# XiangLi2022/CM-TTS

Measured on AMD Instinct MI355X. Metric: mel-frames/s (text->mel hot path, consistency sampling T=4), higher is better.
Workload: dtype f32

## Files before the change

cm-tts_amd/csrc/cmtts_api.hip:

```cpp
#include <hip/hip_runtime.h>
#include <limits.h>
#include <math.h>
#include <stdio.h>
#include <stdlib.h>
#include <string.h>

#include <algorithm>
#include <map>
#include <string>
#include <vector>

#include "../../include/cmtts_hip.h"
#include "internal_hooks.h"
#include "conv_args.h"
#include "kernels.h"
#include "resblock_args.h"
#include "persist_args.h"
#include "cond_gemm.h"
#include "resblock_pair.h"
#include "inproj.h"
#include "attention.h"
#include "text_state.h"

namespace {
// ... 1046 lines not shown
}

struct FrameWs {
    float *xlr, *h128, *hp, *c1, *c2, *cwt, *r, *s1, *s2, *stats, *f0;
    int64_t* pidx;
    size_t bytes;
};
FrameWs carve_frame(const cmtts_config& c, int B, int T, void* base) {
    Carver cv(base);
    FrameWs w;
    const size_t n = (size_t)B * c.hidden * T;
    w.xlr = cv.take<float>(n);
    w.h128 = cv.take<float>((size_t)B * c.cwt_hidden * T);
    w.hp = cv.take<float>((size_t)B * c.cwt_hidden * T);
    w.c1 = cv.take<float>(n);
    w.c2 = cv.take<float>(n);
    w.cwt = cv.take<float>((size_t)B * T * 16);
    w.r = cv.take<float>((size_t)B * T);
    w.s1 = cv.take<float>((size_t)B * c.cwt_hidden);
    w.s2 = cv.take<float>((size_t)B * c.cwt_hidden);
    w.stats = cv.take<float>((size_t)B * 2);
    w.f0 = cv.take<float>((size_t)B * T);
    w.pidx = cv.take<int64_t>((size_t)B * T);
    w.bytes = cv.off + 256;
    return w;
}

struct DenWs {
    float *hin, *h, *u, *zb, *skip, *emb, *e1, *e2, *dproj, *sproj, *dp, *tbuf, *xcur, *cp;
    float* pst;
    unsigned long long* halo;
    size_t bytes;
};
DenWs carve_den(const cmtts_config& c, int B, int T, void* base) {
    Carver cv(base);
    DenWs w;
    const int C = c.res_channels, NL = c.res_layers;
    const size_t n = (size_t)B * C * T;
    w.hin = cv.take<float>((size_t)B * c.n_mels * T);
    w.h = cv.take<float>(n);
    w.u = cv.take<float>(n);
    w.zb = cv.take<float>(n);
    w.skip = cv.take<float>(n);
    w.emb = cv.take<float>((size_t)B * C);
    w.e1 = cv.take<float>((size_t)B * 4 * C);
    w.e2 = cv.take<float>((size_t)B * C);
    w.dproj = cv.take<float>((size_t)B * NL * C);
    w.sproj = cv.take<float>((size_t)B * NL * C);
    w.dp = cv.take<float>((size_t)B * NL * C);
    w.tbuf = cv.take<float>((size_t)B);
    w.xcur = cv.take<float>((size_t)B * T * c.n_mels);
    w.cp = cv.take<float>((size_t)NL * n);
    w.halo = cv.take<unsigned long long>(cmtts_persist_halo_bytes(B, T) / sizeof(unsigned long long));
    w.pst = cv.take<float>(cmtts_persist_state_floats(B, T));
    w.bytes = cv.off + 256;
    return w;
}

struct EnergyHead {
    const float* xin; const float* e_target; float e_control; const float* bins; int nbins; const float* E; float* out1; int64_t* e_idx; float* e_scaled;
    bool done;
};
int g_energy_head = 1;
int g_pred_wino = 1;
int g_pred_xres = 1;
int predictor(const Predictor& P, const float* in, int ld_in, int B, int T, int ld, const int64_t* ln_lens,
              const int64_t* out_lens, float* bufA, float* bufB, float* out, int O, hipStream_t s, int mode16 = 0, bool frame_level = false,
              EnergyHead* eh = nullptr) {
    const float* cur = in;
    int ldc = ld_in;
    auto other = [&](const float* p) { return p == bufA ? bufB : bufA; };
    int pend_ln = -1;
    for (size_t li = 0; li < P.convs.size(); ++li) {
        const PackedConv& w = P.convs[li];
        int rx = -2;
        float* dst = other(cur);
        if (frame_level && !mode16 && g_pred_wino && !ln_lens && li < P.convs_q.size() && P.convs_q[li] && w.taps == 5 && w.cout == 256 &&
            (pend_ln < 0 || w.cin == 256)) {
            ConvXlArgs xa;
            memset(&xa, 0, sizeof(xa));
            xa.x = cur; xa.y = dst; xa.wf = P.convs_q[li]; xa.bias = w.bias; xa.bstride = (long)w.cout * ld;
            xa.B = B; xa.C = 256; xa.T = T; xa.ld = ld; xa.k = w.taps; xa.dil = 1; xa.slope = 1.0f; xa.relu = 1;
            if (w.cin != 256) { xa.cin = w.cin; xa.xbstride = (long)w.cin * ldc; }
            if (pend_ln >= 0) { xa.ln_g = P.ln_g[pend_ln]; xa.ln_b = P.ln_b[pend_ln]; xa.ln_eps = 1e-12f; }
            if (ldc == ld || w.cin != 256) {
                rx = cmtts_launch_conv_k5q(&xa, (void*)s);
                if (rx == -3) return fail(CMTTS_E_HIP, "conv_k5q launch failed");
                if (rx == 0) pend_ln = -2;
            }
        }
        const bool small = (long)((T + 63) / 64) * B < 192;
        if (rx != 0 && !mode16 && g_pred_xres && small && P.convs_f[li] && w.cin == 256 && w.cout == 256 && ldc == ld) {
            ConvArgs a = conv_args(w, cur, T, ldc, (long)w.cin * ldc, dst, ld, (long)w.cout * ld, T);
            a.out[0].act = ACT_RELU;
            a.xres_nt = 1;
            if (pend_ln >= 0) { a.ln_g = P.ln_g[pend_ln]; a.ln_b = P.ln_b[pend_ln]; a.ln_eps = 1e-12f; a.ln_lens = ln_lens; a.ln_skip_tiles = 1; }
            rx = cmtts_launch_conv_xres(&a, P.convs_f[li], B, (void*)s);
            if (rx == -3) return fail(CMTTS_E_HIP, "conv_xres launch failed");
            if (rx == 0) pend_ln = -2;
        }
        if (pend_ln >= 0) {
            float* nd = other(cur);
            k_layernorm_ct(cur, nd, P.ln_g[pend_ln], P.ln_b[pend_ln], 1e-12f, ln_lens, B, T, ld, s);
            cur = nd;
            dst = other(cur);
        }
        pend_ln = -1;
        if (mode16 && li < P.convs_f16[mode16 - 1].size() && P.convs_f16[mode16 - 1][li]) {
            ConvArgs a = conv_args(w, cur, T, ldc, (long)w.cin * ldc, dst, ld, (long)w.cout * ld, T);
            a.out[0].act = ACT_RELU;
            a.text_epi = 1;
            rx = cmtts_launch_conv16(&a, P.convs_f16[mode16 - 1][li], mode16, B, (void*)s);
            if (rx == -3) return fail(CMTTS_E_HIP, "text16: predictor conv launch failed");
        }
        if (rx != 0 && g_pred_xl && P.convs_f[li] && ldc == ld && (long)((T + 63) / 64) * B >= 192) {
            ConvXlArgs xa;
            memset(&xa, 0, sizeof(xa));
            xa.x = cur; xa.y = dst; xa.wf = P.convs_f[li]; xa.bias = w.bias; xa.bstride = (long)w.cout * ld;
            xa.B = B; xa.C = 256; xa.T = T; xa.ld = ld; xa.k = w.taps; xa.dil = 1; xa.slope = 1.0f; xa.relu = 1;
            if (w.cin != 256) { xa.cin = w.cin; xa.xbstride = (long)w.cin * ldc; }
            rx = cmtts_launch_conv_xl(&xa, (void*)s);
            if (rx == -3) return fail(CMTTS_E_HIP, "conv_xl launch failed");
        }
        if (rx != 0) {
            ConvArgs a = conv_args(w, cur, T, ldc, (long)w.cin * ldc, dst, ld, (long)w.cout * ld, T);
            a.out[0].act = ACT_RELU;
            CHK(launch(a, EPI_PLAIN, B, s));
        }
        cur = dst;
        ldc = ld;
        if (g_pred_head && eh && g_energy_head && O == 1 && li + 1 == P.convs.size() && w.cout == 256) {
            k_ln_linear_energy(cur, P.ln_g[li], P.ln_b[li], 1e-12f, P.lin_w, P.lin_b, out, ln_lens, out_lens, B, T, ld, eh->xin, eh->e_target, eh->e_control,
                               eh->bins, eh->nbins, eh->E, eh->out1, eh->e_idx, eh->e_scaled, s);
            eh->done = true;
            return 0;
        }
        if (g_pred_head && li + 1 == P.convs.size() && w.cout == 256 &&
            k_ln_linear(cur, P.ln_g[li], P.ln_b[li], 1e-12f, P.lin_w, P.lin_b, out, ln_lens, out_lens, B, T, ld, O, s))
            return 0;
        pend_ln = (int)li;
    }
    if (pend_ln >= 0) {
        float* nd = other(cur);
        k_layernorm_ct(cur, nd, P.ln_g[pend_ln], P.ln_b[pend_ln], 1e-12f, ln_lens, B, T, ld, s);
        cur = nd;
    }
    k_chan_linear(cur, P.lin_w, P.lin_b, out, out_lens, B, P.convs.back().cout, T, ld, O, s);
    return 0;
}

int cond_projections(cmtts_model* m, const DenWs& w, const float* cond_ct, int B, int T, hipStream_t s) {
    const cmtts_config& c = m->cfg;
    if (g_cond_gemm16 && m->precision >= 1 && m->precision <= 3 && m->cond_all_f16[m->precision - 1]) {
        CondGemmArgs g;
        g.X = cond_ct; g.Wf = nullptr; g.bias = m->cond_all.bias; g.Y = w.cp;
        g.row_split = 0;
        g.B = B; g.T = T; g.M = c.res_layers * c.res_channels; g.K = c.hidden; g.force = 1;
        const int r = cmtts_launch_cond_gemm16(&g, m->cond_all_f16[m->precision - 1], m->precision, (void*)s);
        if (r == 0) return 0;
        if (r != -2) return fail(CMTTS_E_HIP, "cond_gemm16 launch failed");
    }
    if (m->cond_all_f) {
        CondGemmArgs g;
        g.X = cond_ct; g.Wf = m->cond_all_f; g.bias = m->cond_all.bias; g.Y = w.cp;
        g.row_split = 0;
        g.B = B; g.T = T; g.M = c.res_layers * c.res_channels; g.K = c.hidden; g.force = g_cond_gemm == 2;
        const int r = g_cond_gemm ? cmtts_launch_cond_gemm(&g, (void*)s) : -2;
        if (r == 0) return 0;
        if (r != -2) return fail(CMTTS_E_HIP, "cond_gemm launch failed");
    }
    ConvArgs a = conv_args(m->cond_all, cond_ct, T, T, (long)c.hidden * T, w.cp, T, (long)c.res_layers * c.res_channels * T, T);
    return launch(a, EPI_PLAIN, B, s);
}

struct CondFactors {
    const float* p1 = nullptr;
    const float* p1t = nullptr;
    int ldp = 0, L = 0;
    const int64_t* mel2ph = nullptr;
    const int64_t* p_idx = nullptr;
    bool usable(const cmtts_model* m) const;
};
int g_cond_factored = 1;
int g_cond_inkernel = 1;
inline bool C_IS_256(const cmtts_config& c) { return c.res_channels == 256; }
bool CondFactors::usable(const cmtts_model* m) const {
    return g_cond_factored && p1 && mel2ph && p_idx && m->precision == 0 && m->cond_p2 && g_fused_resblock;
}
int cond_factored(cmtts_model* m, const DenWs& w, const CondFactors& f, int B, int T, hipStream_t s) {
    const cmtts_config& c = m->cfg;
    const int r = cmtts_launch_cond_expand(f.p1, f.ldp, f.L, m->cond_p2, c.pitch_bins, f.mel2ph, f.p_idx, w.cp, B, c.res_layers * c.res_channels, T, (void*)s);
    return r == 0 ? 0 : fail(CMTTS_E_HIP, "cond_expand launch failed");
}
int cond_phoneme_factor(cmtts_model* m, const float* out1, int B, int Lp, float* p1, hipStream_t s) {
    const cmtts_config& c = m->cfg;
    if (!m->cond_p2) return fail(CMTTS_E_UNSUPPORTED, "factored conditioner projections are not available for this model");
    CondGemmArgs g;
    memset(&g, 0, sizeof(g));
    g.X = out1; g.Wf = m->cond_all_f; g.bias = m->cond_zero_bias; g.Y = p1;
    g.B = B; g.T = Lp; g.M = c.res_layers * c.res_channels; g.K = c.hidden; g.force = 1;
    g.flat = 1;
    const long tiles = ((long)B * Lp + 63) / 64;
    const int npass = g.M / 512;
    int best = 1;
    double best_t = 1e30;
    for (int sp = 1; sp <= npass; ++sp) {
        const int ppg = (npass + sp - 1) / sp, groups = (npass + ppg - 1) / ppg;
        const long wg = tiles * groups, cap = persist_blocks();
        const double t = (double)((wg + cap - 1) / cap) * ppg;
        if (t < best_t - 1e-9) { best_t = t; best = sp; }
    }
    g.row_split = best;
    const int r = cmtts_launch_cond_gemm(&g, (void*)s);
    return r == 0 ? 0 : fail(r == -2 ? CMTTS_E_UNSUPPORTED : CMTTS_E_HIP, "cond_gemm (phoneme factor) launch failed");
}

int step_embedding(cmtts_model* m, const DenWs& w, const float* timesteps, const float* spk, int B, hipStream_t s,
                   float t_host = NAN) {
    const cmtts_config& c = m->cfg;
    const int C = c.res_channels, NL = c.res_layers;
    if (c.multi_speaker && !spk) return fail(CMTTS_E_INVALID, "speaker_emb is required for a multi-speaker model");
    const bool cacheable = g_step_cache && t_host == t_host;
    if (cacheable) {
        for (const cmtts_model::StepRow& e : m->step_rows)
            if (e.t == t_host && hipEventQuery(e.ready) == hipSuccess) {
                k_broadcast_row(e.row, w.dproj, B, NL * C, s);
                if (c.multi_speaker) {
                    k_dense_small(spk, c.hidden, 1, m->sproj_wt, nullptr, nullptr, w.sproj, B, c.hidden, NL * C, DENSE_NONE, s);
                    k_add_rows(w.dproj, w.sproj, w.dp, (long)B * NL * C, s);
                }
                return 0;
            }
    }
    k_diff_embed(timesteps, m->omega_res, w.emb, B, C, s);
    k_dense_small(w.emb, C, 1, m->mlp0_wt, nullptr, nullptr, w.e1, B, C, 4 * C, DENSE_MISH, s);
    k_dense_small(w.e1, 4 * C, 1, m->mlp2_wt, nullptr, nullptr, w.e2, B, 4 * C, C, DENSE_NONE, s);
    k_dense_small(w.e2, C, 1, m->dproj_wt, nullptr, nullptr, w.dproj, B, C, NL * C, DENSE_NONE, s);
    if (c.multi_speaker) {
        k_dense_small(spk, c.hidden, 1, m->sproj_wt, nullptr, nullptr, w.sproj, B, c.hidden, NL * C, DENSE_NONE, s);
        k_dense_small(w.e2, C, 1, m->dproj_wt, nullptr, w.sproj, w.dp, B, C, NL * C, DENSE_NONE, s);
    }
    if (cacheable && m->step_rows.size() < 16) {
        bool known = false;
        for (const cmtts_model::StepRow& e : m->step_rows) known = known || e.t == t_host;
        if (!known) {
            cmtts_model::StepRow e{t_host, nullptr, nullptr};
            void* p = nullptr;
            if (hipMalloc(&p, (size_t)NL * C * sizeof(float)) == hipSuccess && hipEventCreateWithFlags(&e.ready, hipEventDisableTiming) == hipSuccess) {
                e.row = (float*)p;
                m->al.ptrs.push_back(p);
                HIPCHK(hipMemcpyAsync(e.row, w.dproj, (size_t)NL * C * sizeof(float), hipMemcpyDeviceToDevice, s));
                HIPCHK(hipEventRecord(e.ready, s));
                m->step_rows.push_back(e);
            } else if (p) {
                (void)hipFree(p);
            }
        }
    }
    return 0;
}

struct MelPost {
    const float* xold;
    const float* noise;
    float c_out, c_skip, nstd;
    float* out;
};

int denoiser_prologue(cmtts_model* m, const DenWs& w, const float* x_src, float in_scale, const float* timesteps, const float* spk, int B,
                      int T, hipStream_t s, bool embed, float t_host, bool* halo_zeroed) {
    const cmtts_config& c = m->cfg;
    const int C = c.res_channels, NL = c.res_layers, M = c.n_mels;
    const long cs = (long)C * T;
    *halo_zeroed = false;
    int rin = -2;
    if (g_inproj_fused && m->in_proj_f) {
        InProjArgs ia;
        memset(&ia, 0, sizeof(ia));
        ia.x = x_src; ia.scale = in_scale; ia.wf = m->in_proj_f; ia.bias = m->in_proj.bias; ia.h = w.h;
        ia.B = B; ia.T = T; ia.M = M; ia.C = C;
        const bool persist_path = g_fused_resblock && g_persist && NL <= PERSIST_MAX_LAYERS;
        if (persist_path) { ia.zero = w.halo; ia.zero_f4 = (long)(cmtts_persist_halo_bytes(B, T) / 16); }
        rin = cmtts_launch_inproj(&ia, (void*)s);
        if (rin == -3) return fail(CMTTS_E_HIP, "inproj launch failed");
        *halo_zeroed = rin == 0 && persist_path && cmtts_persist_halo_bytes(B, T) % 16 == 0;
    }
    if (rin != 0) {
        k_mel_prep(x_src, nullptr, in_scale, w.hin, B, T, M, s);
        ConvArgs a = conv_args(m->in_proj, w.hin, T, T, (long)M * T, w.h, T, cs, T);
        a.out[0].act = ACT_RELU;
        CHK(launch(a, EPI_PLAIN, B, s));
    }
    if (embed) CHK(step_embedding(m, w, timesteps, spk, B, s, t_host));
    return 0;
}

int denoiser_core(cmtts_model* m, const DenWs& w, const float* x_src, float in_scale, const float* timesteps,
                  const float* cond_ct, const float* spk, int B, int T, const MelPost& post, hipStream_t s, bool embed = true,
                  SideStream* pending = nullptr, float t_host = NAN,
                  const CondFactors* cfk = nullptr, bool* cp_ready = nullptr) {
    CHK(check_device_flag(true));
    const cmtts_config& c = m->cfg;
    const int C = c.res_channels, NL = c.res_layers, M = c.n_mels;
    const long cs = (long)C * T;
    bool halo_zeroed = false;
    CHK(denoiser_prologue(m, w, x_src, in_scale, timesteps, spk, B, T, s, embed, t_host, &halo_zeroed));
    if (pending) CHK(branch_join(pending));
    const float* dp = m->cfg.multi_speaker ? w.dp : w.dproj;
    const bool unfused = !g_fused_resblock;
    float* hcur = w.h;
    float* halt = w.u;
    bool layers_done = false;
    if (!unfused && g_persist && NL <= PERSIST_MAX_LAYERS) {
        PersistArgs pa;
        memset(&pa, 0, sizeof(pa));
        pa.x0 = w.h; pa.cp = w.cp; pa.cp_bstride = (long)NL * C * T;
        pa.dp = dp; pa.d = w.dproj; pa.vec_stride = (long)NL * C;
        pa.skip = w.skip; pa.halo = w.halo; pa.tmo = g_tmo_host;
        pa.B = B; pa.T = T; pa.NL = NL;
        pa.halo_zeroed = halo_zeroed;
        const int prec = m->precision;
        if (cfk && !(cp_ready && *cp_ready)) {
            pa.fact = 1; pa.p1 = cfk->p1; pa.p2 = m->cond_p2; pa.mel2ph = (const long long*)cfk->mel2ph; pa.pidx = (const long long*)cfk->p_idx;
            pa.ldp = cfk->ldp; pa.Lph = cfk->L; pa.ld2 = c.pitch_bins;
            pa.p1t = cfk->p1t; pa.p2t = m->cond_p2t;
        }
        if (g_persist_tail && m->skip_f && m->outp_f) {
            pa.tail = 1;
            pa.Wsf = m->skip_f; pa.bs = m->skip_proj.bias; pa.Wpf = m->outp_f; pa.bp = m->out_proj.bias;
            pa.skip_div = (float)sqrt((double)NL); pa.n_mels = M;
            pa.xold = post.xold; pa.noise = post.noise; pa.c_out = post.c_out; pa.c_skip = post.c_skip; pa.nstd = post.nstd;
            pa.out = post.out;
        }
        pa.wino = g_persist_wino && m->winograd && !prec && m->res[0].w3w && w.pst;
        if (pa.wino && g_persist_wino == 3 && m->winograd == 1 && m->res[0].w3w43) pa.wino = 3;
        pa.xst = w.pst;
        for (int l = 0; l < NL; ++l) {
            pa.W3f[l] = prec ? (const float*)m->res[l].w3f16[prec - 1] : (pa.wino == 3 ? m->res[l].w3w43 : pa.wino ? m->res[l].w3w : m->res[l].w3f);
            pa.Wof[l] = prec ? (const float*)m->res[l].wof16[prec - 1] : m->res[l].wof;
            pa.b3[l] = m->res[l].b3f; pa.bo[l] = m->res[l].outp.bias;
        }
        const bool prof = g_prof.on && g_prof.used + 2 <= g_prof.ev.size();
        const int need = cmtts_persist_plan(B, T, NL, persist_blocks(), g_persist == 2);
        if (need) CHK(persist_admit(s, need, persist_blocks()));
        if (prof) (void)hipEventRecord(g_prof.ev[g_prof.used], s);
        const int rc = prec ? cmtts_launch_denoiser_persist_lp(&pa, prec, persist_blocks(), g_persist == 2, (void*)s)
                            : cmtts_launch_denoiser_persist(&pa, persist_blocks(), g_persist == 2, (void*)s);
        if (rc == -3) return fail(CMTTS_E_HIP, "persistent denoiser launch failed");
        if (rc == 0) {
            CHK(persist_launched(s, need));
            if (prof) { (void)hipEventRecord(g_prof.ev[g_prof.used + 1], s); g_prof.used += 2; }
            layers_done = true;
            if (pa.tail) return 0;
        }
    }
    if (!layers_done && cfk && !(cp_ready && *cp_ready)) {
        CHK(cond_factored(m, w, *cfk, B, T, s));
        if (cp_ready) *cp_ready = true;
    }
    for (int l = 0; l < NL && !layers_done; ++l) {
        const ResLayer& R = m->res[l];
        const bool prof = g_prof.on && g_prof.used + 2 <= g_prof.ev.size() && (g_prof.seen++ % g_prof.stride) == 0;
        if (!unfused) {
            ResArgs ra;
            memset(&ra, 0, sizeof(ra));
            ra.x_in = hcur; ra.cp = w.cp + (long)l * C * T; ra.cp_bstride = (long)NL * C * T;
// ... 237 lines not shown
            ConvArgs a = conv_args(E.ffn1, ln_ffn ? w.x : w.h, L, Lp, hs, w.f, Lp, 4 * hs, L);
            a.out[0].alpha = (float)pow((double)c.ffn_kernel, -0.5);
            a.out[0].act = ACT_GELU_ERF;
            if (ln_ffn) { a.ln_g = E.ln2_g; a.ln_b = E.ln2_b; a.ln_eps = 1e-12f; a.ln_lens = pad_lens; a.ln_skip_tiles = pad_lens != nullptr; }
            int rc = -2;
            if (xr && g_ffn_fused && ffn2_seg && E.ffn2_f && E.ffn1.cout == FFN2_SEG * 128) {
                a.w2frag = E.ffn2_f; a.part = w.part; a.part_zs0 = (long)FFN2_SEG * hs; a.part_zs1 = hs; a.part_ld = Lp; a.M2 = H;
                rc = wq ? cmtts_launch_conv_xresq(&a, wqf, B, (void*)s, g_ffn_wino == 2 ? 1 : 2) : -2;
                if (rc == -2) rc = cmtts_launch_conv_xres(&a, E.ffn1_f, B, (void*)s);
                if (rc == 0) ffn_fused = true;
                else { a.w2frag = nullptr; a.part = nullptr; }
            }
            if (xr && !ffn_fused) rc = cmtts_launch_conv_xres(&a, E.ffn1_f, B, (void*)s);
            if (rc == -3) return fail(CMTTS_E_HIP, "conv_xres launch failed");
            if (rc != 0) {
                if (ln_ffn) {
                    k_layernorm_ct(w.x, w.h, E.ln2_g, E.ln2_b, 1e-12f, pad_lens, B, L, Lp, s);
                    a.X = w.h; a.ln_g = a.ln_b = nullptr; a.ln_lens = nullptr;
                }
                CHK(launch(a, EPI_PLAIN, B, s));
            }
        }
        if (ffn_fused) {
            k_reduce_partials(w.part, FFN2_SEG, E.ffn2.bias, w.x, src_lens, w.x, B, H, L, Lp, s);
        } else if (ffn2_seg) {
            const int kseg = E.ffn2.cin / FFN2_SEG;
            ConvArgs a = conv_args(E.ffn2, w.f, L, Lp, 4 * hs, w.part, Lp, (long)FFN2_SEG * hs, L);
            a.K = kseg;
            a.zdiv = FFN2_SEG; a.a_zs0 = 0; a.a_zs1 = (long)kseg * a.a_ld; a.x_zs1 = (long)kseg * Lp;
            a.out[0].y_zs1 = hs; a.out[0].bias = nullptr;
            CHK(launch(a, EPI_PLAIN, B * FFN2_SEG, s));
            k_reduce_partials(w.part, FFN2_SEG, E.ffn2.bias, w.x, src_lens, w.x, B, H, L, Lp, s);
        } else {
            ConvArgs a = conv_args(E.ffn2, w.f, L, Lp, 4 * hs, w.x, Lp, hs, L);
            a.out[0].res = w.x; a.out[0].r_zs0 = hs; a.out[0].ldr = Lp; a.out[0].lens = src_lens;
            CHK(launch(a, EPI_PLAIN, B, s));
        }
    }
    return 0;
}

int cmtts_text_forward(cmtts_model* m, const int64_t* texts, const int64_t* src_lens, const float* spker_embeds,
                       const int64_t* speakers, int B, int L, float d_control, float* log_d, float* d_rounded, int64_t* mel_len,
                       float* e_pred, int64_t* e_idx, float* enc_out_ct, float* speaker_emb,
                       void* text_ws, size_t text_ws_bytes, void* stream) {
    return cmtts_text_forward_ragged(m, texts, src_lens, nullptr, spker_embeds, speakers, B, L, d_control, log_d, d_rounded, mel_len, e_pred,
                                     e_idx, enc_out_ct, speaker_emb, text_ws, text_ws_bytes, stream);
}

int cmtts_text_forward_ragged(cmtts_model* m, const int64_t* texts, const int64_t* src_lens, const int64_t* pad_lens, const float* spker_embeds,
                              const int64_t* speakers, int B, int L, float d_control, float* log_d, float* d_rounded, int64_t* mel_len,
                              float* e_pred, int64_t* e_idx, float* enc_out_ct, float* speaker_emb,
                              void* text_ws, size_t text_ws_bytes, void* stream) {
    if (!m || !m->finalized) return fail(CMTTS_E_INVALID, "model not finalized");
    if (!texts || !src_lens || !text_ws || B <= 0 || L <= 0) return fail(CMTTS_E_INVALID, "cmtts_text_forward: bad argument");
    const cmtts_config& c = m->cfg;
    if (c.multi_speaker && c.n_speaker > 0 && !speakers) return fail(CMTTS_E_INVALID, "speakers (ids into the speaker_emb table) are required (model/cmtts.py:78)");
    if (c.multi_speaker && c.n_speaker <= 0 && !spker_embeds) return fail(CMTTS_E_INVALID, "Speaker embedding should not be None (model/cmtts.py:80)");
    TextWs w = carve_text(c, B, L, text_ws);
    if (text_ws_bytes < w.bytes) return fail(CMTTS_E_WORKSPACE, "text workspace too small");
    hipStream_t s = (hipStream_t)stream;
    const int H = c.hidden, Lp = round_up(L, 4);
    if (!log_d) log_d = w.logd;
    if (!d_rounded) d_rounded = w.dround;
    if (!mel_len) mel_len = w.mlen;
    if (!e_pred) e_pred = w.epred;
    if (!e_idx) e_idx = w.eidx;

    k_embed_tokens(texts, src_lens, m->embed, m->omega_h, m->pe_h, PE_ROWS, w.x, B, L, Lp, H, (float)sqrt((double)H), s);
    CHK(fft_stack(m, m->enc, w, src_lens, B, L, s, pad_lens));
    k_layernorm_ct(w.x, w.x, m->encln_g, m->encln_b, 1e-5f, src_lens, B, L, Lp, s);
    if (enc_out_ct && c.multi_speaker)
        k_copy_rows(enc_out_ct, L, w.x, Lp, L, (long)B * H, s);
    if (c.multi_speaker) {
        if (c.n_speaker > 0) k_gather_rows(m->spk_table, speakers, w.spk, B, H, c.n_speaker, s);
        else k_dense_small(spker_embeds, c.external_speaker_dim, 1, m->spk_wt, m->spk_b, nullptr, w.spk, B,
                      c.external_speaker_dim, H, DENSE_NONE, s);
        k_add_rowvec(w.x, w.spk, B, H, L, Lp, s, pad_lens);
        if (speaker_emb) HIPCHK(hipMemcpyAsync(speaker_emb, w.spk, (size_t)B * H * 4, hipMemcpyDeviceToDevice, s));
    }
    SideStream* ss = side_for(s);
    hipStream_t se = ss ? ss->side : s;
    float* ec1 = ss ? w.qk : w.c1;
    float* ec2 = ss ? w.qk + (size_t)B * H * Lp : w.c2;
    if (ss) CHK(branch_fork(ss));
    const int t16mode = (m->text16 && (m->precision == 1 || m->precision == 2)) ? m->precision : 0;
    CHK(predictor(m->dur, w.x, Lp, B, L, Lp, src_lens, src_lens, w.c1, w.c2, log_d, 1, s, t16mode));
    if (m->vc.d_target) {
        HIPCHK(hipMemcpyAsync(d_rounded, m->vc.d_target, (size_t)B * L * 4, hipMemcpyDeviceToDevice, s));
        k_cumsum_durations(m->vc.d_target, w.cum, mel_len, B, L, s);
    } else {
        k_durations(log_d, d_control, d_rounded, w.cum, mel_len, B, L, s);
    }
    if (enc_out_ct && !c.multi_speaker)
        k_copy_rows(enc_out_ct, L, w.x, Lp, L, (long)B * H, s);
    k_pos_embed_add(w.x, w.h, m->energy.alpha, m->omega_h, m->pe_h, PE_ROWS, B, H, L, Lp, se);
    EnergyHead eh{w.x, m->vc.e_target, m->vc.e_control, m->energy_bins, c.energy_bins - 1, m->energy_emb, w.out1, e_idx, w.escaled, false};
    CHK(predictor(m->energy, w.h, Lp, B, L, Lp, pad_lens, pad_lens, ec1, ec2, e_pred, 1, se, t16mode, false, H == 256 ? &eh : nullptr));
    if (ss) CHK(branch_join(ss));
    if (!eh.done)
        k_energy_embed(w.x, e_pred, w.escaled, m->vc.e_target, m->vc.e_control, m->energy_bins, c.energy_bins - 1, m->energy_emb,
                       w.out1, e_idx, B, H, L, Lp, s);
    {
        ConvArgs a = conv_args(m->cwt_in, w.out1, L, Lp, (long)H * Lp, w.h128, Lp, (long)c.cwt_hidden * Lp, L);
        int rc = -2;
        if (g_ffn_xres && g_pred_xres && m->cwt_in_f) {
            a.xres_nt = 1;
            rc = cmtts_launch_conv_xres(&a, m->cwt_in_f, B, (void*)s);
            if (rc == -3) return fail(CMTTS_E_HIP, "conv_xres launch failed");
            a.xres_nt = 0;
        }
        if (rc != 0) CHK(launch(a, EPI_PLAIN, B, s));
    }
    if (!m->vc.e_target && m->vc.e_control != 1.0f)
        HIPCHK(hipMemcpyAsync(e_pred, w.escaled, (size_t)B * L * 4, hipMemcpyDeviceToDevice, s));
    HIPCHK(hipGetLastError());
    return 0;
}

int cmtts_frame_forward(cmtts_model* m, const void* text_ws, int B, int L, int T, float* cond_ct, int64_t* mel2ph,
                        float* cwt_out, float* f0_denorm, int64_t* p_idx, float* f0_stats, void* frame_ws,
                        size_t frame_ws_bytes, void* stream) {
    return cmtts_frame_forward_sub(m, text_ws, B, L, 0, B, T, cond_ct, mel2ph, cwt_out, f0_denorm, p_idx, f0_stats, nullptr, frame_ws, frame_ws_bytes, stream);
}

int cmtts_frame_forward_sub(cmtts_model* m, const void* text_ws, int B_all, int L_all, int b0, int B, int T, float* cond_ct, int64_t* mel2ph,
                            float* cwt_out, float* f0_denorm, int64_t* p_idx, float* f0_stats, float* cond_p1, void* frame_ws,
                            size_t frame_ws_bytes, void* stream) {
    return cmtts_frame_forward_sub_t(m, text_ws, B_all, L_all, b0, B, T, cond_ct, mel2ph, cwt_out, f0_denorm, p_idx, f0_stats, cond_p1, nullptr, frame_ws,
                                     frame_ws_bytes, stream);
}

int cmtts_frame_forward_sub_t(cmtts_model* m, const void* text_ws, int B_all, int L_all, int b0, int B, int T, float* cond_ct, int64_t* mel2ph,
                              float* cwt_out, float* f0_denorm, int64_t* p_idx, float* f0_stats, float* cond_p1, float* cond_p1t, void* frame_ws,
                              size_t frame_ws_bytes, void* stream) {
    if (!m || !m->finalized) return fail(CMTTS_E_INVALID, "model not finalized");
    if (!text_ws || !frame_ws || !cond_ct || !mel2ph || B <= 0 || L_all <= 0 || T <= 0 || b0 < 0 || b0 + B > B_all)
        return fail(CMTTS_E_INVALID, "cmtts_frame_forward: bad argument");
    const cmtts_config& c = m->cfg;
    const int L = L_all;
    TextWs tw = carve_text(c, B_all, L_all, const_cast<void*>(text_ws));
    tw.out1 += (size_t)b0 * c.hidden * round_up(L_all, 4);
    tw.h128 += (size_t)b0 * c.cwt_hidden * round_up(L_all, 4);
    tw.cum += (size_t)b0 * L_all;
    FrameWs w = carve_frame(c, B, T, frame_ws);
    if (frame_ws_bytes < w.bytes) return fail(CMTTS_E_WORKSPACE, "frame workspace too small");
    hipStream_t s = (hipStream_t)stream;
    const int H = c.hidden, Lp = round_up(L, 4), O = c.use_uv ? 11 : 10, CH = c.cwt_hidden;
    if (!cwt_out) cwt_out = w.cwt;
    if (!f0_denorm) f0_denorm = w.f0;
    if (!p_idx) p_idx = w.pidx;
    if (!f0_stats) f0_stats = w.stats;

    SideStream* ss = side_for(s);
    hipStream_t sst = ss ? ss->side : s;
    if (ss) CHK(branch_fork(ss));
    if (cond_p1t && !cond_p1) return fail(CMTTS_E_INVALID, "cmtts_frame_forward_sub_t: cond_p1t needs cond_p1");
    if (cond_p1 && m->cond_p2) {
        CHK(cond_phoneme_factor(m, tw.out1, B, Lp, cond_p1, sst));
        if (cond_p1t) k_transpose(cond_p1, cond_p1t, B * c.res_layers, c.res_channels, Lp, sst);
    }
    if (!(g_stats_mlp && k_stats_mlp(tw.out1, (long)H * Lp, Lp, m->st0_wt, m->st0_b, m->st2_wt, m->st2_b, m->st4_wt, m->st4_b, f0_stats, B, H, CH, CH, 2, sst))) {
        k_dense_small(tw.out1, (long)H * Lp, Lp, m->st0_wt, m->st0_b, nullptr, w.s1, B, H, CH, DENSE_RELU, sst);
        k_dense_small(w.s1, CH, 1, m->st2_wt, m->st2_b, nullptr, w.s2, B, CH, CH, DENSE_RELU, sst);
        k_dense_small(w.s2, CH, 1, m->st4_wt, m->st4_b, nullptr, f0_stats, B, CH, 2, DENSE_NONE, sst);
    }
    k_mel2ph(tw.cum, mel2ph, B, L, T, s);
    if (!g_cwt_in_phoneme) k_length_regulate(tw.out1, mel2ph, w.xlr, B, H, Lp, T, s);
    bool hp_done = false;
    if (g_cwt_in_phoneme) {
        k_pos_embed_add_lr(tw.h128, Lp, mel2ph, m->cwt_in.bias, w.hp, m->cwt.alpha, m->omega_cwt, m->pe_cwt, PE_ROWS, B, CH, T, s);
        hp_done = true;
    } else {
        ConvArgs a = conv_args(m->cwt_in, w.xlr, T, T, (long)H * T, w.h128, T, (long)CH * T, T);
        CHK(launch(a, EPI_PLAIN, B, s));
    }
    if (!hp_done) k_pos_embed_add(w.h128, w.hp, m->cwt.alpha, m->omega_cwt, m->pe_cwt, PE_ROWS, B, CH, T, T, s);
    CHK(predictor(m->cwt, w.hp, T, B, T, T, nullptr, nullptr, w.c1, w.c2, cwt_out, O, s, (m->text16 && (m->precision == 1 || m->precision == 2)) ? m->precision : 0, true));
    if (ss) CHK(branch_join(ss));
    if (m->vc.p_control != 1.0f) k_scale(cwt_out, cwt_out, (long)B * T * O, m->vc.p_control, s);
    if (m->vc.cwt_spec) {
        k_pitch_index(m->vc.cwt_spec, 10, m->vc.f0_mean, m->vc.f0_std, 1, 1.0f, nullptr, 0, c.use_uv ? m->vc.uv : nullptr,
                      c.pitch_norm_eps, w.r, p_idx, f0_denorm, B, T, s);
    } else {
        k_pitch_index(cwt_out, O, f0_stats, f0_stats + 1, 2, c.cwt_std_scale, c.use_uv ? cwt_out + (O - 1) : nullptr, O, nullptr,
                      c.pitch_norm_eps, w.r, p_idx, f0_denorm, B, T, s);
    }
    if (g_cwt_in_phoneme) k_lr_gather_add(tw.out1, mel2ph, Lp, p_idx, m->pitch_emb, cond_ct, B, H, T, s);
    else k_gather_add(w.xlr, p_idx, m->pitch_emb, cond_ct, B, H, T, s);
    HIPCHK(hipGetLastError());
    return 0;
}

namespace {
struct TextStateLayout {
    long off[TEXT_STATE_MAX_REGIONS], bytes[TEXT_STATE_MAX_REGIONS], stride[TEXT_STATE_MAX_REGIONS];
    long rec_bytes;
};
TextStateLayout text_state_layout(const cmtts_config& c, int L) {
    const int Lp = round_up(L, 4);
    TextStateLayout t;
    t.bytes[0] = (long)c.hidden * Lp * 4;
    t.bytes[1] = (long)c.cwt_hidden * Lp * 4;
    t.bytes[2] = (long)c.hidden * 4;
    t.bytes[3] = (long)L * 4;
    long off = TEXT_STATE_HEADER_BYTES;
    for (int g = 0; g < TEXT_STATE_MAX_REGIONS; ++g) {
        t.stride[g] = t.bytes[g];
        t.off[g] = off;
        off += (t.bytes[g] + 15) / 16 * 16;
    }
    t.rec_bytes = off;
    return t;
}
TextStateCopy text_state_args(const cmtts_config& c, void* ws, int B_all, int L, void* records, int n, int unpack) {
    const TextStateLayout t = text_state_layout(c, L);
    TextWs tw = carve_text(c, B_all, L, ws);
    char* base[TEXT_STATE_MAX_REGIONS] = {(char*)tw.out1, (char*)tw.h128, (char*)tw.spk, (char*)tw.cum};
    TextStateCopy a;
    memset(&a, 0, sizeof(a));
    int chunks = 0;
    for (int g = 0; g < TEXT_STATE_MAX_REGIONS; ++g) {
        TextStateRegion& R = a.reg[g];
        R.ws = base[g]; R.ws_stride = t.stride[g]; R.rec_off = t.off[g]; R.bytes = t.bytes[g];
        R.vec16 = ((uintptr_t)R.ws % 16 == 0 && R.ws_stride % 16 == 0 && R.bytes % 16 == 0 && (uintptr_t)records % 16 == 0) ? 1 : 0;
        R.chunk0 = chunks;
        chunks += (int)((R.bytes + TEXT_STATE_CHUNK - 1) / TEXT_STATE_CHUNK);
    }
    a.n_regions = TEXT_STATE_MAX_REGIONS; a.n_chunks = chunks; a.unpack = unpack;
    a.n = n; a.B_all = B_all; a.L_all = L; a.hidden = c.hidden; a.cwt_hidden = c.cwt_hidden;
    a.rec = (char*)records; a.rec_bytes = t.rec_bytes;
    a.cum = tw.cum;
    return a;
}
}

size_t cmtts_text_state_record_bytes(const cmtts_model* m, int L_all) {
    if (!m || L_all <= 0) return 0;
    return (size_t)text_state_layout(m->cfg, L_all).rec_bytes;
}

int cmtts_text_state_pack(cmtts_model* m, const void* text_ws, int B_all, int L_all, const int32_t* rows, int n, const int64_t* global_idx,
                          const int64_t* src_lens, void* records, void* stream) {
    if (!m || !m->finalized) return fail(CMTTS_E_INVALID, "model not finalized");
    if (!text_ws || !records || (n > 0 && !rows) || B_all <= 0 || L_all <= 0 || n < 0)
        return fail(CMTTS_E_INVALID, "cmtts_text_state_pack: bad argument");
    if ((uintptr_t)records % 16) return fail(CMTTS_E_INVALID, "cmtts_text_state_pack: records must be 16-byte aligned");
    TextStateCopy a = text_state_args(m->cfg, const_cast<void*>(text_ws), B_all, L_all, records, n, 0);
    a.rows = rows; a.index = global_idx; a.src_lens = src_lens;
    if (cmtts_launch_text_state_copy(&a, stream) != 0) return fail(CMTTS_E_HIP, "text-state pack launch failed");
    return 0;
}

int cmtts_text_state_unpack(cmtts_model* m, const void* records, int n, int L_all, void* text_ws, size_t text_ws_bytes, void* stream) {
    if (!m || !m->finalized) return fail(CMTTS_E_INVALID, "model not finalized");
    if (!text_ws || !records || n <= 0 || L_all <= 0) return fail(CMTTS_E_INVALID, "cmtts_text_state_unpack: bad argument");
    if ((uintptr_t)records % 16) return fail(CMTTS_E_INVALID, "cmtts_text_state_unpack: records must be 16-byte aligned");
    if (text_ws_bytes < carve_text(m->cfg, n, L_all, nullptr).bytes) return fail(CMTTS_E_WORKSPACE, "text workspace too small");
    TextStateCopy a = text_state_args(m->cfg, text_ws, n, L_all, const_cast<void*>(records), n, 1);
    if (cmtts_launch_text_state_copy(&a, stream) != 0) return fail(CMTTS_E_HIP, "text-state unpack launch failed");
    return 0;
}

int cmtts_length_regulate(const float* x_ct, const float* durations, int B, int C, int L, int T, float* out_ct,
                          int64_t* mel2ph, int64_t* mel_len, int32_t* scratch_cum, void* stream) {
    if (!x_ct || !durations || !out_ct || !mel2ph || !mel_len || !scratch_cum || B <= 0 || L <= 0 || T <= 0)
        return fail(CMTTS_E_INVALID, "cmtts_length_regulate: bad argument");
    hipStream_t s = (hipStream_t)stream;
    k_cumsum_durations(durations, scratch_cum, mel_len, B, L, s);
    k_mel2ph(scratch_cum, mel2ph, B, L, T, s);
    k_length_regulate(x_ct, mel2ph, out_ct, B, C, L, T, s);
    HIPCHK(hipGetLastError());
    return 0;
}

int cmtts_denoiser_forward(cmtts_model* m, const float* x, const float* timesteps, const float* cond_ct,
                           const float* speaker_emb, int B, int T, float* out, void* ws, size_t ws_bytes, void* stream) {
    if (!m || !m->finalized) return fail(CMTTS_E_INVALID, "model not finalized");
    if (!x || !timesteps || !cond_ct || !out || !ws || B <= 0 || T <= 0)
        return fail(CMTTS_E_INVALID, "cmtts_denoiser_forward: bad argument");
    DenWs w = carve_den(m->cfg, B, T, ws);
    if (ws_bytes < w.bytes) return fail(CMTTS_E_WORKSPACE, "denoiser workspace too small");
    hipStream_t s = (hipStream_t)stream;
    SideStream* ss = g_fused_resblock ? side_for(s) : nullptr;
    if (ss) CHK(branch_fork(ss));
    if (g_fused_resblock) CHK(cond_projections(m, w, cond_ct, B, T, ss ? ss->side : s));
    const MelPost post = {nullptr, nullptr, 1.0f, 0.0f, 0.0f, out};
    CHK(denoiser_core(m, w, x, 1.0f, timesteps, cond_ct, speaker_emb, B, T, post, s, true, ss));
    HIPCHK(hipGetLastError());
    return 0;
}

int cmtts_schedule(const cmtts_model* m, int n_steps, float* sigmas, float* renoise_std) {
    if (!m || !sigmas || !renoise_std || n_steps < 1) return fail(CMTTS_E_INVALID, "cmtts_schedule: bad argument");
    const cmtts_config& c = m->cfg;
    if (n_steps == 1) {
        sigmas[0] = c.sigma_max;
        renoise_std[0] = -1.0f;
        return 0;
    }
    const double rho = c.rho, tmax = pow((double)c.sigma_max, 1.0 / rho), tmin = pow((double)c.sigma_min, 1.0 / rho);
    for (int i = 0; i < n_steps; ++i) {
        const double tsi = 0.0, tsn = (i + 1 == n_steps) ? 1.0 : 0.0;
        const double t = pow(tmax + tsi / 1.0 * (tmin - tmax), rho);
        double nt = pow(tmax + tsn / 1.0 * (tmin - tmax), rho);
        nt = nt < c.sigma_min ? (double)c.sigma_min : (nt > c.sigma_max ? (double)c.sigma_max : nt);
        sigmas[i] = (float)t;
        renoise_std[i] = (float)sqrt(nt * nt - (double)c.sigma_min * (double)c.sigma_min);
    }
    return 0;
}

}
namespace {
int sample_core(cmtts_model* m, const DenWs& w, const float* noise, long noise_stride, const float* cond_ct, const float* speaker_emb, int B,
                int T, int n_steps, const float* sigmas, const float* renoise_std, float* mel, hipStream_t s, const CondFactors* cf = nullptr) {
    const cmtts_config& c = m->cfg;
    const long nel = (long)B * T * c.n_mels;
    SideStream* ss = g_fused_resblock ? side_for(s) : nullptr;
    if (ss) CHK(branch_fork(ss));
    const CondFactors* cfk = nullptr;
    CondFactors cf_local;
    bool cp_ready = false;
    if (g_fused_resblock) {
        if (cf && cf->usable(m)) {
            const bool inkernel = g_cond_inkernel && g_persist && g_persist_tail && m->skip_f && m->outp_f && c.res_layers <= PERSIST_MAX_LAYERS &&
                                  cmtts_persist_plan(B, T, c.res_layers, persist_blocks(), g_persist == 2) > 0;
            if (inkernel && cf->ldp <= T && m->cond_p2t && C_IS_256(c)) {
                cf_local = *cf;
                if (!cf_local.p1t) {
// ... 900 lines not shown
```

cm-tts_amd/csrc/cond_gemm.h:

```cpp
#pragma once

struct CondGemmArgs {
    const float* X;
    const float* Wf;
    const float* bias;
    float* Y;
    int B, T, M, K;
    int force;
    int flat;
    int row_split;
};

#ifdef __cplusplus
extern "C" {
#endif
int cmtts_launch_cond_gemm(const CondGemmArgs* a, void* stream);
int cmtts_launch_cond_expand(const float* p1, int ldp, int L, const float* p2, int ld2, const int64_t* mel2ph, const int64_t* pidx,
                             float* cp, int B, int M, int T, void* stream);
int cmtts_launch_cond_gemm16(const CondGemmArgs* a, const void* wf16, int mode, void* stream);
#ifdef __cplusplus
}
#endif
```

cm-tts_amd/csrc/cond_gemm.hip:

```cpp
#include <hip/hip_runtime.h>
#include "cond_gemm.h"

typedef float f32x16 __attribute__((ext_vector_type(16)));
typedef float f32x4 __attribute__((ext_vector_type(4)));

namespace {

constexpr int K = 256;
constexpr int NW = 8;
constexpr int MT = 2;
constexpr int FN = 64;
constexpr int NT = FN / 32;
constexpr int X_LD = FN + 4;
constexpr int RING = 4;
constexpr int NG = K / 8;

__device__ __forceinline__ float ldg(const float* base, unsigned idx) {
    return *reinterpret_cast<const float*>(reinterpret_cast<const char*>(base) + (size_t)(idx * 4u));
}
__device__ __forceinline__ int acc_row(int r, int lane) { return (r & 3) + 8 * (r >> 2) + 4 * (lane >> 5); }

__global__ __launch_bounds__(64 * NW, 2) void cond_gemm_kernel(const CondGemmArgs a) {
    extern __shared__ __attribute__((aligned(16))) float xs[];
    const int tid = threadIdx.x, lane = tid & 63, w = tid >> 6;
    const int t0 = blockIdx.x * FN;
    const int l31 = lane & 31, khalf = lane >> 5;
    const int T = a.T;
    const long ncol = a.flat ? (long)a.B * T : T;
    auto col_x = [&](long c) -> long { return a.flat ? (c / T) * (long)K * T + (c % T) : (long)blockIdx.y * K * T + c; };
    auto col_y = [&](long c) -> long { return a.flat ? (c / T) * (long)a.M * T + (c % T) : (long)blockIdx.y * a.M * T + c; };
    const float* xin = a.X;
    float* yb = a.Y;

    {
        const long t = t0 + lane;
        const long xo = col_x(t < ncol ? t : ncol - 1);
#pragma unroll 1
        for (int i = 0; i < K / NW; i += 8) {
            float xv[8];
#pragma unroll
            for (int q = 0; q < 8; ++q) xv[q] = xin[xo + (long)(w * (K / NW) + i + q) * T];
#pragma unroll
            for (int q = 0; q < 8; ++q) xs[(w * (K / NW) + i + q) * X_LD + lane] = t < ncol ? xv[q] : 0.f;
        }
    }
    const int MTn = a.M / 32;
    auto load_a = [&](f32x4 (&dst)[MT], int mt0, int g) {
#pragma unroll
        for (int i = 0; i < MT; ++i)
            dst[i] = *reinterpret_cast<const f32x4*>(a.Wf + (((long)g * MTn + mt0 + i) * 64 + lane) * 4);
    };
    auto load_b = [&](float (&dst)[4][NT], int g) {
        const float* bs = xs + (g * 8 + khalf) * X_LD + l31;
#pragma unroll
        for (int kk = 0; kk < 4; ++kk)
#pragma unroll
            for (int j = 0; j < NT; ++j) dst[kk][j] = bs[2 * kk * X_LD + j * 32];
    };
    const int npass_all = a.M / (32 * MT * NW);
    const int ppg = (npass_all + (int)gridDim.z - 1) / (int)gridDim.z;
    const int p_first = (int)blockIdx.z * ppg;
    const int npass = min(npass_all, p_first + ppg);
    if (p_first >= npass) return;
    f32x4 A[RING][MT];
#pragma unroll
    for (int s = 0; s < RING - 1; ++s) load_a(A[s], (p_first * NW + w) * MT, s);
    __syncthreads();

    for (int p = p_first; p < npass; ++p) {
        const int mt0 = (p * NW + w) * MT;
        f32x16 acc[MT][NT];
#pragma unroll
        for (int i = 0; i < MT; ++i)
#pragma unroll
            for (int j = 0; j < NT; ++j)
#pragma unroll
                for (int r = 0; r < 16; ++r) acc[i][j][r] = 0.f;
        float Bv[2][4][NT];
        load_b(Bv[0], 0);
        const int mt_next = (min(p + 1, npass - 1) * NW + w) * MT;
#pragma unroll 1
        for (int it = 0; it < NG; it += RING) {
#pragma unroll
            for (int s = 0; s < RING; ++s) {
                const int nx = it + s + RING - 1;
                if (nx < NG) load_a(A[(s + RING - 1) % RING], mt0, nx);
                else load_a(A[(s + RING - 1) % RING], mt_next, nx - NG);
                load_b(Bv[(s + 1) & 1], min(it + s + 1, NG - 1));
                __builtin_amdgcn_sched_barrier(0);
#pragma unroll
                for (int kk = 0; kk < 4; ++kk)
#pragma unroll
                    for (int i = 0; i < MT; ++i)
#pragma unroll
                        for (int j = 0; j < NT; ++j)
                            acc[i][j] = __builtin_amdgcn_mfma_f32_32x32x2f32(A[s][i][kk], Bv[s & 1][kk][j], acc[i][j], 0, 0, 0);
                __builtin_amdgcn_sched_barrier(0);
            }
        }
#pragma unroll
        for (int i = 0; i < MT; ++i) {
            const int m0 = (mt0 + i) * 32;
            float bi[16];
#pragma unroll
            for (int r = 0; r < 16; ++r) bi[r] = ldg(a.bias, (unsigned)(m0 + acc_row(r, lane)));
#pragma unroll
            for (int j = 0; j < NT; ++j) {
                const long t = t0 + j * 32 + l31;
                const long yo = col_y(t < ncol ? t : ncol - 1);
#pragma unroll
                for (int r = 0; r < 16; ++r)
                    if (t < ncol) yb[yo + (long)(m0 + acc_row(r, lane)) * T] = acc[i][j][r] + bi[r];
            }
        }
    }
}

}

extern "C" int cmtts_launch_cond_gemm(const CondGemmArgs* ap, void* stream_) {
    const CondGemmArgs& a = *ap;
    if (a.K != K || a.M % (32 * MT * NW) != 0 || (long)a.M * a.T >= (1L << 30) || a.B <= 0 || a.T <= 0) return -2;
    if (a.flat && (long)a.B * a.T >= (1L << 30)) return -2;
    if (!a.force && (long)((a.T + FN - 1) / FN) * a.B < 128) return -2;
    static bool attr_set = false;
    const size_t lds = (size_t)K * X_LD * sizeof(float);
    if (!attr_set) {
        if (hipFuncSetAttribute(reinterpret_cast<const void*>(cond_gemm_kernel), hipFuncAttributeMaxDynamicSharedMemorySize,
                                (int)lds) != hipSuccess)
            return -3;
        attr_set = true;
    }
    const int zsplit = a.row_split > 1 ? a.row_split : 1;
    const dim3 grid = a.flat ? dim3((unsigned)(((long)a.B * a.T + FN - 1) / FN), 1, zsplit) : dim3((a.T + FN - 1) / FN, a.B, zsplit);
    hipLaunchKernelGGL(cond_gemm_kernel, grid, dim3(64 * NW), lds, (hipStream_t)stream_, a);
    return hipGetLastError() == hipSuccess ? 0 : -3;
}

namespace {
constexpr int CEX_ROWS = 64;
template <int V>
__global__ __launch_bounds__(256) void cond_expand_kernel(const float* __restrict__ p1, int ldp, int L, const float* __restrict__ p2, int ld2,
                                                          const int64_t* __restrict__ mel2ph, const int64_t* __restrict__ pidx,
                                                          float* __restrict__ cp, int M, int T) {
    const int t = (blockIdx.x * 64 + (threadIdx.x & 63)) * V;
    const int r0 = blockIdx.y * CEX_ROWS + (threadIdx.x >> 6) * (CEX_ROWS / 4), b = blockIdx.z;
    if (t >= T) return;
    int ph[V], ix[V];
#pragma unroll
    for (int e = 0; e < V; ++e) {
        const int64_t p64 = mel2ph[(long)b * T + t + e];
        ph[e] = (int)(p64 > L ? L : p64);
        const int i = (int)pidx[(long)b * T + t + e];
        ix[e] = i < 0 ? 0 : (i >= ld2 ? ld2 - 1 : i);
    }
    const float* a = p1 + ((long)b * M + r0) * ldp;
    const float* q = p2 + (long)r0 * ld2;
    float* o = cp + ((long)b * M + r0) * T + t;
#pragma unroll 1
    for (int r = 0; r < CEX_ROWS / 4; r += 4) {
        float av[4][V], qv[4][V];
#pragma unroll
        for (int j = 0; j < 4; ++j)
#pragma unroll
            for (int e = 0; e < V; ++e) {
                av[j][e] = a[(long)(r + j) * ldp + (ph[e] > 0 ? ph[e] - 1 : 0)];
                qv[j][e] = q[(long)(r + j) * ld2 + ix[e]];
            }
#pragma unroll
        for (int j = 0; j < 4; ++j) {
            if (V == 4) {
                f32x4 v;
#pragma unroll
                for (int e = 0; e < 4; ++e) v[e] = (ph[e] > 0 ? av[j][e] : 0.f) + qv[j][e];
                *reinterpret_cast<f32x4*>(o + (long)(r + j) * T) = v;
            } else {
                o[(long)(r + j) * T] = (ph[0] > 0 ? av[j][0] : 0.f) + qv[j][0];
            }
        }
    }
}
}

extern "C" int cmtts_launch_cond_expand(const float* p1, int ldp, int L, const float* p2, int ld2, const int64_t* mel2ph, const int64_t* pidx,
                                        float* cp, int B, int M, int T, void* stream_) {
    if (M % CEX_ROWS != 0 || B <= 0 || T <= 0 || L <= 0) return -2;
    if ((T & 3) == 0 && ((uintptr_t)cp & 15) == 0)
        hipLaunchKernelGGL(cond_expand_kernel<4>, dim3((T / 4 + 63) / 64, M / CEX_ROWS, B), dim3(256), 0, (hipStream_t)stream_, p1, ldp, L, p2, ld2,
                           mel2ph, pidx, cp, M, T);
    else
        hipLaunchKernelGGL(cond_expand_kernel<1>, dim3((T + 63) / 64, M / CEX_ROWS, B), dim3(256), 0, (hipStream_t)stream_, p1, ldp, L, p2, ld2,
                           mel2ph, pidx, cp, M, T);
    return hipGetLastError() == hipSuccess ? 0 : -3;
}
```

Baseline: 1.972 million.

## Fuse phoneme-factor transpose into cond GEMM epilogue and delay side-stream fork

The conditioner GEMM epilogue now also writes a transposed copy of its output (Yt) with vectorized stores, which removes the separate transpose kernel. If the fused path is rejected, it falls back to the old GEMM plus transpose. The side-stream fork carrying the phoneme factor and stats MLP is moved later, after the length-regulate and positional-embed work, so the side branch overlaps with the CWT predictor instead of competing with the earlier main-stream kernels. Risks are extra store traffic and register pressure in the GEMM epilogue, and less overlap for the early main-stream work.

```diff
diff --git a/cm-tts_amd/csrc/cmtts_api.hip b/cm-tts_amd/csrc/cmtts_api.hip
--- a/cm-tts_amd/csrc/cmtts_api.hip
+++ b/cm-tts_amd/csrc/cmtts_api.hip
@@ -1222,7 +1222,7 @@
 int cond_projections(cmtts_model* m, const DenWs& w, const float* cond_ct, int B, int T, hipStream_t s) {
     const cmtts_config& c = m->cfg;
     if (g_cond_gemm16 && m->precision >= 1 && m->precision <= 3 && m->cond_all_f16[m->precision - 1]) {
-        CondGemmArgs g;
+        CondGemmArgs g{};
         g.X = cond_ct; g.Wf = nullptr; g.bias = m->cond_all.bias; g.Y = w.cp;
         g.row_split = 0;
         g.B = B; g.T = T; g.M = c.res_layers * c.res_channels; g.K = c.hidden; g.force = 1;
@@ -1231,7 +1231,7 @@
         if (r != -2) return fail(CMTTS_E_HIP, "cond_gemm16 launch failed");
     }
     if (m->cond_all_f) {
-        CondGemmArgs g;
+        CondGemmArgs g{};
         g.X = cond_ct; g.Wf = m->cond_all_f; g.bias = m->cond_all.bias; g.Y = w.cp;
         g.row_split = 0;
         g.B = B; g.T = T; g.M = c.res_layers * c.res_channels; g.K = c.hidden; g.force = g_cond_gemm == 2;
@@ -1262,7 +1262,7 @@
     const int r = cmtts_launch_cond_expand(f.p1, f.ldp, f.L, m->cond_p2, c.pitch_bins, f.mel2ph, f.p_idx, w.cp, B, c.res_layers * c.res_channels, T, (void*)s);
     return r == 0 ? 0 : fail(CMTTS_E_HIP, "cond_expand launch failed");
 }
-int cond_phoneme_factor(cmtts_model* m, const float* out1, int B, int Lp, float* p1, hipStream_t s) {
+int cond_phoneme_factor(cmtts_model* m, const float* out1, int B, int Lp, float* p1, hipStream_t s, float* p1t = nullptr) {
     const cmtts_config& c = m->cfg;
     if (!m->cond_p2) return fail(CMTTS_E_UNSUPPORTED, "factored conditioner projections are not available for this model");
     CondGemmArgs g;
@@ -1270,6 +1270,7 @@
     g.X = out1; g.Wf = m->cond_all_f; g.bias = m->cond_zero_bias; g.Y = p1;
     g.B = B; g.T = Lp; g.M = c.res_layers * c.res_channels; g.K = c.hidden; g.force = 1;
     g.flat = 1;
+    g.Yt = p1t; g.Ct = c.res_channels;
     const long tiles = ((long)B * Lp + 63) / 64;
     const int npass = g.M / 512;
     int best = 1;
@@ -1281,7 +1282,12 @@
         if (t < best_t - 1e-9) { best_t = t; best = sp; }
     }
     g.row_split = best;
-    const int r = cmtts_launch_cond_gemm(&g, (void*)s);
+    int r = cmtts_launch_cond_gemm(&g, (void*)s);
+    if (r == -2 && p1t) {
+        g.Yt = nullptr;
+        r = cmtts_launch_cond_gemm(&g, (void*)s);
+        if (r == 0) k_transpose(p1, p1t, B * c.res_layers, c.res_channels, Lp, s);
+    }
     return r == 0 ? 0 : fail(r == -2 ? CMTTS_E_UNSUPPORTED : CMTTS_E_HIP, "cond_gemm (phoneme factor) launch failed");
 }
 
@@ -1825,19 +1831,7 @@
     if (!p_idx) p_idx = w.pidx;
     if (!f0_stats) f0_stats = w.stats;
 
-    SideStream* ss = side_for(s);
-    hipStream_t sst = ss ? ss->side : s;
-    if (ss) CHK(branch_fork(ss));
     if (cond_p1t && !cond_p1) return fail(CMTTS_E_INVALID, "cmtts_frame_forward_sub_t: cond_p1t needs cond_p1");
-    if (cond_p1 && m->cond_p2) {
-        CHK(cond_phoneme_factor(m, tw.out1, B, Lp, cond_p1, sst));
-        if (cond_p1t) k_transpose(cond_p1, cond_p1t, B * c.res_layers, c.res_channels, Lp, sst);
-    }
-    if (!(g_stats_mlp && k_stats_mlp(tw.out1, (long)H * Lp, Lp, m->st0_wt, m->st0_b, m->st2_wt, m->st2_b, m->st4_wt, m->st4_b, f0_stats, B, H, CH, CH, 2, sst))) {
-        k_dense_small(tw.out1, (long)H * Lp, Lp, m->st0_wt, m->st0_b, nullptr, w.s1, B, H, CH, DENSE_RELU, sst);
-        k_dense_small(w.s1, CH, 1, m->st2_wt, m->st2_b, nullptr, w.s2, B, CH, CH, DENSE_RELU, sst);
-        k_dense_small(w.s2, CH, 1, m->st4_wt, m->st4_b, nullptr, f0_stats, B, CH, 2, DENSE_NONE, sst);
-    }
     k_mel2ph(tw.cum, mel2ph, B, L, T, s);
     if (!g_cwt_in_phoneme) k_length_regulate(tw.out1, mel2ph, w.xlr, B, H, Lp, T, s);
     bool hp_done = false;
@@ -1849,6 +1843,17 @@
         CHK(launch(a, EPI_PLAIN, B, s));
     }
     if (!hp_done) k_pos_embed_add(w.h128, w.hp, m->cwt.alpha, m->omega_cwt, m->pe_cwt, PE_ROWS, B, CH, T, T, s);
+    SideStream* ss = side_for(s);
+    hipStream_t sst = ss ? ss->side : s;
+    if (ss) CHK(branch_fork(ss));
+    if (cond_p1 && m->cond_p2) {
+        CHK(cond_phoneme_factor(m, tw.out1, B, Lp, cond_p1, sst, cond_p1t));
+    }
+    if (!(g_stats_mlp && k_stats_mlp(tw.out1, (long)H * Lp, Lp, m->st0_wt, m->st0_b, m->st2_wt, m->st2_b, m->st4_wt, m->st4_b, f0_stats, B, H, CH, CH, 2, sst))) {
+        k_dense_small(tw.out1, (long)H * Lp, Lp, m->st0_wt, m->st0_b, nullptr, w.s1, B, H, CH, DENSE_RELU, sst);
+        k_dense_small(w.s1, CH, 1, m->st2_wt, m->st2_b, nullptr, w.s2, B, CH, CH, DENSE_RELU, sst);
+        k_dense_small(w.s2, CH, 1, m->st4_wt, m->st4_b, nullptr, f0_stats, B, CH, 2, DENSE_NONE, sst);
+    }
     CHK(predictor(m->cwt, w.hp, T, B, T, T, nullptr, nullptr, w.c1, w.c2, cwt_out, O, s, (m->text16 && (m->precision == 1 || m->precision == 2)) ? m->precision : 0, true));
     if (ss) CHK(branch_join(ss));
     if (m->vc.p_control != 1.0f) k_scale(cwt_out, cwt_out, (long)B * T * O, m->vc.p_control, s);
diff --git a/cm-tts_amd/csrc/cond_gemm.h b/cm-tts_amd/csrc/cond_gemm.h
--- a/cm-tts_amd/csrc/cond_gemm.h
+++ b/cm-tts_amd/csrc/cond_gemm.h
@@ -9,6 +9,8 @@
     int force;
     int flat;
     int row_split;
+    float* Yt;
+    int Ct;
 };
 
 #ifdef __cplusplus
diff --git a/cm-tts_amd/csrc/cond_gemm.hip b/cm-tts_amd/csrc/cond_gemm.hip
--- a/cm-tts_amd/csrc/cond_gemm.hip
+++ b/cm-tts_amd/csrc/cond_gemm.hip
@@ -111,6 +111,18 @@
 #pragma unroll
                 for (int r = 0; r < 16; ++r)
                     if (t < ncol) yb[yo + (long)(m0 + acc_row(r, lane)) * T] = acc[i][j][r] + bi[r];
+                if (a.Yt && t < ncol) {
+                    const long b = t / T, tt = t - b * T;
+                    const int g = m0 / a.Ct, ch0 = m0 - g * a.Ct + 4 * khalf;
+                    float* yt = a.Yt + ((b * (a.M / a.Ct) + g) * T + tt) * a.Ct + ch0;
+#pragma unroll
+                    for (int q = 0; q < 4; ++q) {
+                        f32x4 v;
+#pragma unroll
+                        for (int e = 0; e < 4; ++e) v[e] = acc[i][j][4 * q + e] + bi[4 * q + e];
+                        *reinterpret_cast<f32x4*>(yt + 8 * q) = v;
+                    }
+                }
             }
         }
     }
@@ -122,6 +134,7 @@
     const CondGemmArgs& a = *ap;
     if (a.K != K || a.M % (32 * MT * NW) != 0 || (long)a.M * a.T >= (1L << 30) || a.B <= 0 || a.T <= 0) return -2;
     if (a.flat && (long)a.B * a.T >= (1L << 30)) return -2;
+    if (a.Yt && (!a.flat || a.Ct <= 0 || a.Ct % 32 != 0 || a.M % a.Ct != 0 || ((uintptr_t)a.Yt & 15) != 0)) return -2;
     if (!a.force && (long)((a.T + FN - 1) / FN) * a.B < 128) return -2;
     static bool attr_set = false;
     const size_t lds = (size_t)K * X_LD * sizeof(float);
```

Measured after the change: 1.976 million (median of 6 runs). No clear change (+0.2%).
